# pauxy-qmc/pauxy

Measured on AMD Instinct MI355X. Metric: walker_steps_per_sec, higher is better.
Workload: dtype f64; 1 GPU; generic Cholesky AFQMC: Nbasis=100, Nchol=500, RHF trial 25+25 electrons, 256 walkers/GPU, dt=0.005, reortho/10, comb/5, energy/10 (BASELINE configs[2]); walkers_total=256, rng=device-philox, population_control=device comb (one rank)

## Files before the change

include/afqmc_hip.h:

```cpp
#ifndef AFQMC_HIP_H
#define AFQMC_HIP_H

#include <stdint.h>

#ifdef __cplusplus
extern "C" {
#endif

typedef struct afq_handle afq_handle;

#define AFQ_OK            0
#define AFQ_EINVAL       (-1)
#define AFQ_ESTATE       (-2)
#define AFQ_EHIP         (-3)
#define AFQ_ENOMEM       (-4)
#define AFQ_EUNSUPPORTED (-5)
#define AFQ_EWEIGHT      (-6)
#define AFQ_EOVERFLOW    (-7)
#define AFQ_ECOMM        (-8)

#define AFQ_SYS_GENERIC 1
#define AFQ_SYS_HUBBARD 2
#define AFQ_SYS_UEG     3

// ... 103 lines not shown
int afq_propagate_begin(afq_handle *h, const double *xi);
int afq_propagate_finish(afq_handle *h, double eshift_re, double eshift_im);
int afq_reortho(afq_handle *h, double *detR_out);
int afq_set_log_shift(afq_handle *h, int on, double log_shift, double detR_shift);
int afq_log_ovlp_sums(afq_handle *h, double *sums3);
int afq_local_energy(afq_handle *h, double *E_out);

int afq_set_exchange_algorithm(afq_handle *h, int mode);
int afq_exchange_algorithm(afq_handle *h, int *mode_out);

int afq_set_propagator_closed_form(afq_handle *h, int mode);
int afq_propagator_closed_form(afq_handle *h, int *mode_out);

int afq_set_step_fusion(afq_handle *h, int mode);
int afq_set_step_fusion_scope(afq_handle *h, int scope);

int afq_set_msd_force_bias(afq_handle *h, int mode);
int afq_msd_force_bias(afq_handle *h, int *mode_out);

int afq_force_bias(afq_handle *h, double *xbar_out);
int afq_shift_fields(afq_handle *h, const double *xi, const double *xbar,
                     double *xs_out, double *cmf_out, double *cfb_out);
int afq_vhs(afq_handle *h, const double *xs, double *vhs_out);
int afq_vhs_count(afq_handle *h, int *nv);
int afq_apply_exponential(afq_handle *h, const double *vhs);
int afq_kinetic(afq_handle *h);

int afq_cap_weights(afq_handle *h, double frac, double total_weight);
int afq_set_weight_cap(afq_handle *h, double frac, double total_weight);
int afq_popcontrol_comb(afq_handle *h, double r, double target_weight,
// ... 89 lines not shown
```

pauxy_amd/_lib.py:

```python
import ctypes
import os
from ctypes import POINTER, c_char_p, c_double, c_int, c_int32, c_int64, c_uint64, c_void_p

HERE = os.path.dirname(os.path.abspath(__file__))
LIB_PATH = os.environ.get("AFQ_LIBRARY") or os.path.join(HERE, "libafqmc_hip.so")

AFQ_OK = 0
AFQ_EWEIGHT, AFQ_EOVERFLOW, AFQ_ECOMM = -6, -7, -8
AFQ_COMM_NSTATS = 12
ALLGATHER_FN = ctypes.CFUNCTYPE(ctypes.c_int, ctypes.c_void_p, ctypes.c_void_p, ctypes.c_int, ctypes.c_void_p)
AFQ_SYS_GENERIC, AFQ_SYS_HUBBARD, AFQ_SYS_UEG = 1, 2, 3
AFQ_PROP_HYBRID, AFQ_PROP_FORCE_BIAS, AFQ_PROP_FREE_PROJECTION, AFQ_PROP_HUBBARD_SPIN = 1, 2, 4, 8
(F_PHI, F_WEIGHT, F_UNSCALED_WEIGHT, F_OT, F_HYBRID_ENERGY, F_PHASE, F_DETR, F_ELOC, F_GHALF, F_G,
 F_XBAR, F_XSHIFTED, F_ENERGY, F_LOG_DETR, F_THERMAL_G, F_THERMAL_STACK, F_THERMAL_RIGHT, F_THERMAL_M0,
 F_THERMAL_DET, F_CMF, F_CFB) = range(21)
THERMAL_CHARGE, THERMAL_FREE_PROJECTION, THERMAL_LOW_RANK, THERMAL_AVERAGE_GF = 1, 2, 4, 8
AFQ_EINVAL, AFQ_ESTATE, AFQ_EUNSUPPORTED = -1, -2, -5

_h = c_void_p
_dp = c_void_p
_ip = c_void_p

SIGNATURES = {
    "afq_version": [],
# ... 97 lines not shown
    "afq_comm_set_timeout": [_h, c_double],
    "afq_launch_trace": [_h, c_int],
    "afq_launch_trace_get": [_h, c_void_p, c_int, c_void_p, c_void_p, c_int, POINTER(c_int)],
    "afq_comm_stats": [_h, c_void_p],
    "afq_comm_parent_ix": [_h, c_void_p],
    "afq_estimates_allreduce": [_h, _dp, c_int],
    "afq_comm_init_local": [POINTER(_h), c_int],
    "afq_popcontrol_comb_local": [POINTER(_h), c_int, c_double, c_double, c_void_p, POINTER(c_double)],
    "afq_estimates_allreduce_local": [POINTER(_h), c_int],
    "afq_set_exchange_algorithm": [_h, c_int],
    "afq_exchange_algorithm": [_h, POINTER(c_int)],
    "afq_set_propagator_closed_form": [_h, c_int],
    "afq_propagator_closed_form": [_h, POINTER(c_int)],
    "afq_set_step_fusion": [_h, c_int],
    "afq_set_step_fusion_scope": [_h, c_int],
    "afq_set_msd_force_bias": [_h, c_int],
    "afq_msd_force_bias": [_h, POINTER(c_int)],
    "afq_kernel_trace": [_h, c_int],
    "afq_kernel_trace_stride": [_h, c_int, c_int],
    "afq_kernel_trace_get": [_h, c_int, _dp, c_int, POINTER(c_int)],
    "afq_kernel_issued_flops": [_h, c_int, POINTER(c_double)],
    "afq_thermal_configure": [_h, c_int, c_int, c_int, _dp, _dp, _dp, _dp, c_int],
    "afq_thermal_reset": [_h],
    "afq_thermal_propagate": [_h, _dp, c_void_p, c_double],
    "afq_thermal_greens": [_h, c_int],
    "afq_thermal_energy": [_h, _dp, _dp],
    "afq_thermal_state": [_h, c_void_p],
    "afq_thermal_configure_continuous": [_h, c_int, c_int, c_double, _dp, _dp, _dp, _dp, c_double, c_int],
    "afq_thermal_propagate_continuous": [_h, _dp, _dp],
}
# ... 41 lines not shown
```

pauxy_amd/csrc/afq_api.hip:

```cpp
#include <algorithm>
#include <cmath>
#include <complex>
#include <cstdio>
#include <cstdlib>
#include <cstring>
#include "afq_host.h"
#include "walker_fields.h"

namespace {

void free_dets(afq_handle *h) {
    h->mem.release(LT_TRIAL);
    h->dets.assign(1, afq_handle::DetOps());
    h->ndet = 1;
    select_det(h, 0, true);
    h->msd_fb_gbar = false;
}

void free_system(afq_handle *h) {
    free_dets(h);
    h->mem.release(LT_SYSTEM);
    h->hs_cplx = 0; h->sf_nlong = 0; h->kind = 0; h->pair_nb = 0;
    h->hirsch = false;
}
// ... 24 lines not shown
                const double hr = hrow[2 * q], hi = hrow[2 * q + 1];
                out[2 * q] += cr * hr - ci * hi;
                out[2 * q + 1] += cr * hi + ci * hr;
            }
        }
    }
    int rc = dev_upload(h, LT_TRIAL, &h->dets[h->cur_det].rH1, r.data(), (size_t)nt * M);
    select_det(h, h->cur_det, true);
    return rc;
}

}

struct afq_host_cache {
    std::vector<double> H1, psi;
};
static afq_host_cache *cache_of(afq_handle *h);

struct afq_handle_full : afq_handle {
    afq_host_cache cache;
};
static afq_host_cache *cache_of(afq_handle *h) { return &static_cast<afq_handle_full *>(h)->cache; }

static int upload_psi(afq_handle *h, const double *psi) {
    const size_t n = (size_t)h->M * h->nt;
    afq_handle::DetOps &o = h->dets[h->cur_det];
    int rc = dev_upload(h, LT_TRIAL, &o.psi, psi, n);
    if (rc) return rc;
    cache_of(h)->psi.assign(psi, psi + 2 * n);
    h->psi_real = true;
    for (size_t i = 0; i < n && h->psi_real; ++i) h->psi_real = psi[2 * i + 1] == 0.0;
    h->psi_closed = h->na == h->nb && h->na > 0;
    for (int p_ = 0; p_ < h->M && h->psi_closed; ++p_)
        h->psi_closed = memcmp(psi + 2 * (size_t)p_ * h->nt, psi + 2 * ((size_t)p_ * h->nt + h->na), sizeof(double) * 2 * h->na) == 0;
    std::vector<double> pc(psi, psi + 2 * n);
    for (size_t i = 0; i < n; ++i) pc[2 * i + 1] = -pc[2 * i + 1];
    if (h->ndet <= 1) {
        std::vector<double> pt(2 * n);
        for (int p_ = 0; p_ < h->M; ++p_)
            for (int i = 0; i < h->nt; ++i) {
                pt[2 * ((size_t)i * h->M + p_)] = pc[2 * ((size_t)p_ * h->nt + i)];
                pt[2 * ((size_t)i * h->M + p_) + 1] = pc[2 * ((size_t)p_ * h->nt + i) + 1];
            }
        if ((rc = dev_upload(h, LT_TRIAL, &h->psicT, pt.data(), n))) return rc;
    }
    rc = dev_upload(h, LT_TRIAL, &o.psic, pc.data(), n);
    select_det(h, h->cur_det, true);
    return rc;
}

static int maybe_build_rH1(afq_handle *h) {
    afq_host_cache *c = cache_of(h);
    if (h->kind == 0 || !h->have_trial || c->H1.empty()) return AFQ_OK;
    return build_rH1(h, c->H1, c->psi);
}

__global__ void afq_marker_kernel(volatile unsigned long long *retired, unsigned long long n) { *retired = n; }

void afq_launch_trace_mark(afq_handle *h, const char *name) {
    const size_t pairs = h->ltrace_name.size();
    if (name && pairs >= 65536) return;
    auto event_at = [&](size_t i) {
// ... 405 lines not shown
    }
    return AFQ_OK;
}

int afq_set_propagator(afq_handle *h, const double *BH1, const double *mf_shift, double dt, int exp_order,
                       int flags) {
    if (h) h->gf.drop();
    if (!h || !BH1 || !mf_shift || dt <= 0 || exp_order < 0) return AFQ_EINVAL;
    if (!h->kind) AFQ_FAIL(h, AFQ_ESTATE, "set the system before the propagator");
    hipSetDevice(h->device);
    int rc;
    if ((rc = dev_upload(h, LT_HANDLE, &h->BH1, BH1, (size_t)2 * h->M * h->M))) return rc;
    h->bh1_real = true;
    h->bh1_same = memcmp(BH1, BH1 + (size_t)2 * h->M * h->M, sizeof(double) * 2 * h->M * h->M) == 0;
    for (size_t i = 0, n = (size_t)2 * h->M * h->M; i < n && h->bh1_real; ++i) h->bh1_real = BH1[2 * i + 1] == 0.0;
    if ((rc = dev_upload(h, LT_HANDLE, &h->mf_shift, mf_shift, (size_t)h->K))) return rc;
    if (h->kind == AFQ_SYS_UEG && (rc = k_ueg_fast_propagator(h, BH1))) return rc;
    h->dt = dt; h->sqrt_dt = std::pow(dt, 0.5); h->exp_order = exp_order;
    if (flags & AFQ_PROP_FREE_PROJECTION) flags &= ~AFQ_PROP_FORCE_BIAS;
    const int old_nv = h->nv; const bool old_diag = h->vhs_diag;
    h->flags = flags;
    h->vhs_diag = h->kind == AFQ_SYS_HUBBARD;
    h->nv = (h->kind == AFQ_SYS_HUBBARD && (flags & AFQ_PROP_HUBBARD_SPIN)) ? 2 : 1;
    h->have_prop = true;
    if (h->nw && (old_nv != h->nv || old_diag != h->vhs_diag || !h->vhs)) {
        const size_t per = h->vhs_diag ? (size_t)2 * h->nv * h->M : (size_t)h->nv * h->M * h->M;
        if ((rc = dev_alloc(h, LT_WALKERS, &h->vhs, per * h->nw))) return rc;
    }
    return AFQ_OK;
}

int afq_walkers_alloc(afq_handle *h, int nw) {
    if (h) h->gf.drop();
    if (!h || nw <= 0) return AFQ_EINVAL;
    if (!h->kind) AFQ_FAIL(h, AFQ_ESTATE, "set the system before allocating walkers");
    hipSetDevice(h->device);
    free_walkers(h);
    const size_t per = (size_t)h->M * h->nt, K = h->K, n = nw;
    int rc = 0;
// ... 492 lines not shown
    return AFQ_OK;
}

int afq_set_step_fusion(afq_handle *h, int mode) {
    if (!h || mode < 0 || mode > 2) return AFQ_EINVAL;
    h->step_fusion_mode = mode;
    return AFQ_OK;
}

int afq_set_step_fusion_scope(afq_handle *h, int scope) {
    if (!h || scope < 0 || scope > 1) return AFQ_EINVAL;
    h->step_fusion_scope = scope;
    return AFQ_OK;
}

int afq_propagator_closed_form(afq_handle *h, int *mode) {
    if (!h || !mode) return AFQ_EINVAL;
    *mode = k_prop_closed_resident(h) ? 2 : 1;
    return AFQ_OK;
}

int afq_set_msd_force_bias(afq_handle *h, int mode) {
    if (!h || mode < 0 || mode > 2) return AFQ_EINVAL;
    h->msd_fb_mode = mode;
    return AFQ_OK;
}

int afq_msd_force_bias(afq_handle *h, int *mode) {
    if (!h || !mode) return AFQ_EINVAL;
    if (h->kind != AFQ_SYS_GENERIC || !h->have_trial || !h->nw) AFQ_FAIL(h, AFQ_ESTATE, "generic system, trial and walkers must be set");
// ... 517 lines not shown
    if (!h->hirsch) AFQ_FAIL(h, AFQ_ESTATE, "the discrete Hirsch propagator is not set");
    return hirsch_buffers(h);
}

int afq_set_propagator_hirsch(afq_handle *h, const double *bt2, double dt, int charge_decomposition) {
    if (h) h->gf.drop();
    if (!h || !bt2 || dt <= 0) return AFQ_EINVAL;
    if (h->kind != AFQ_SYS_HUBBARD) AFQ_FAIL(h, AFQ_ESTATE, "the Hirsch transformation needs a Hubbard system");
    if (h->ndet > 1) AFQ_FAIL(h, AFQ_EUNSUPPORTED, "Hirsch propagator: single-determinant trials");
    hipSetDevice(h->device);
    int rc;
    if ((rc = dev_upload(h, LT_HANDLE, &h->BH1, bt2, (size_t)2 * h->M * h->M))) return rc;
    h->bh1_real = true;
    for (size_t i = 0, n = (size_t)2 * h->M * h->M; i < n && h->bh1_real; ++i) h->bh1_real = bt2[2 * i + 1] == 0.0;
    h->bh1_same = false;
    typedef std::complex<double> C;
    C gamma, auxf[2][2], wfac[2];
    const double e = std::exp(-0.5 * dt * h->U);
    if (charge_decomposition) {
        gamma = std::acosh(C(e, 0.0));
        auxf[0][0] = auxf[0][1] = std::exp(gamma);
        auxf[1][0] = auxf[1][1] = std::exp(-gamma);
        wfac[0] = std::exp(0.5 * dt * h->U) * std::exp(-gamma);
        wfac[1] = std::exp(0.5 * dt * h->U) * std::exp(gamma);
    } else {
        gamma = C(std::acosh(std::exp(0.5 * dt * h->U)), 0.0);
        auxf[0][0] = std::exp(gamma); auxf[0][1] = std::exp(-gamma);
        auxf[1][0] = std::exp(-gamma); auxf[1][1] = std::exp(gamma);
        wfac[0] = wfac[1] = C(1.0, 0.0);
    }
// ... 189 lines not shown
```

pauxy_amd/csrc/afq_internal.h:

```cpp
#pragma once
#include <hip/hip_runtime.h>
#include <stdint.h>
#include <cstdlib>
#include <string>
#include <vector>
#include "../../include/afqmc_hip.h"
#include "greens_cache.h"
#include "dev_mem.h"

typedef double2 cplx;

__host__ __device__ inline cplx cmake(double r, double i) { return make_double2(r, i); }
__host__ __device__ inline cplx cadd(cplx a, cplx b) { return cmake(a.x + b.x, a.y + b.y); }
__host__ __device__ inline cplx csub(cplx a, cplx b) { return cmake(a.x - b.x, a.y - b.y); }
__host__ __device__ inline cplx cmul(cplx a, cplx b) {
    return cmake(a.x * b.x - a.y * b.y, a.x * b.y + a.y * b.x);
}
__host__ __device__ inline cplx cconj(cplx a) { return cmake(a.x, -a.y); }
__host__ __device__ inline cplx cscale(cplx a, double s) { return cmake(a.x * s, a.y * s); }
__host__ __device__ inline void cfma(cplx &a, cplx b, cplx c) {
    a.x = fma(b.x, c.x, a.x); a.x = fma(-b.y, c.y, a.x);
    a.y = fma(b.x, c.y, a.y); a.y = fma(b.y, c.x, a.y);
}
__host__ __device__ inline double cabs2(cplx a) { return a.x * a.x + a.y * a.y; }
__device__ inline cplx cdiv(cplx a, cplx b) {
    if (fabs(b.x) >= fabs(b.y)) {
        double r = b.y / b.x, d = b.x + b.y * r;
        return cmake((a.x + a.y * r) / d, (a.y - a.x * r) / d);
    } else {
        double r = b.x / b.y, d = b.x * r + b.y;
        return cmake((a.x * r + a.y) / d, (a.y * r - a.x) / d);
    }
}

#define AFQ_NSCAL 12
enum { AFQ_HS_HERMITIAN = 1, AFQ_HS_GENERAL = 2 };
enum { T_GREENS = 0, T_ONEBODY, T_FB, T_VHS, T_EXP, T_OVLP, T_QR, T_ENERGY, T_COUNT };

#define AFQ_NCOUNTERS 8

struct afq_handle {
    int device = 0;
    hipStream_t stream = nullptr;
    std::string err;
    DevMem mem;

    int kind = 0;
    int M = 0, K = 0, na = 0, nb = 0, nt = 0;
    double ecore = 0.0;
    double *hs_pot = nullptr;
    bool hs_sym = false;
    double *L_full = nullptr;
    int2 *hs_pair = nullptr;
    int hs_cplx = 0;
// ... 1 lines not shown
    int2 *hs_pair_im = nullptr;
    long ld_hs_im = 0;
    cplx *L_full_c = nullptr;
    long ld_hs = 0, ld_rc = 0;
    bool rchol_real = true;
    double *rchol_re = nullptr;
    double *rchol_im = nullptr;
    double *rchol_frag[2] = {nullptr, nullptr};
    double *rchol_frag_im[2] = {nullptr, nullptr};
    void *atil[2] = {nullptr, nullptr};
    bool atil_unavailable = false;
    bool rchol_same = false;
    int exx_mode = 0;
    int step_fusion_mode = 2;
    int step_fusion_scope = 0;
    int prop_closed_mode = 0;
    cplx *exq_y = nullptr;
    size_t exq_y_len = 0;
    cplx *H1 = nullptr;
    cplx *rH1 = nullptr;
    double U = 0.0;
    int nq = 0;
    int64_t nnzA = 0, nnzB = 0;
    int64_t *iA_colptr = nullptr, *iA_row = nullptr; cplx *iA_val = nullptr;
    int64_t *iB_colptr = nullptr, *iB_row = nullptr; cplx *iB_val = nullptr;
    int64_t *iA_rowptr = nullptr, *iA_col = nullptr; cplx *iA_rval = nullptr;
    int64_t *iB_rowptr = nullptr, *iB_col = nullptr; cplx *iB_rval = nullptr;
    int ell_len = 0; int *ell_row = nullptr; cplx *ell_val = nullptr;
    int ueg_nrows = 0; int *ueg_rmap = nullptr; int *ueg_rows = nullptr;
    int *ueg_kp = nullptr, *ueg_pm = nullptr, *ueg_koff = nullptr, *ueg_poff = nullptr;
// ... 7 lines not shown
    size_t sf_ws_len = 0, sf_two_len = 0;
    cplx *corr_ws = nullptr;
    size_t corr_ws_len = 0;
    int *pair_nbr = nullptr;
    int pair_nb = 0;
    cplx *pair_ws = nullptr;
    size_t pair_ws_len = 0;

    bool have_trial = false;
    cplx *psi = nullptr;
    cplx *psic = nullptr;
    cplx *psicT = nullptr;
    long psi_stride = 0;
    bool psi_real = false;
    bool psi_closed = false;
    unsigned long long *closed_bad = nullptr;
    unsigned long long closed_epoch = 0;
    unsigned long long closed_epoch_pub = 0;
    bool exx_open_hint = false;
    int *closed_w = nullptr;
    size_t closed_w_n = 0;
    bool closed_large = false;

    struct DetOps {
        cplx *psi = nullptr, *psic = nullptr, *rH1 = nullptr;
        double *rchol_re = nullptr, *rchol_im = nullptr;
        double *rchol_frag[2] = {nullptr, nullptr}, *rchol_frag_im[2] = {nullptr, nullptr};
        void *atil[2] = {nullptr, nullptr};
        bool rchol_same = false;
        GreensCache::Stamp vbias_stamp;
// ... 459 lines not shown
```

pauxy_amd/csrc/greens_small.h:

```cpp
#pragma once
#include <type_traits>
#include "mfma_gemm.h"
#include "gj_wave.h"
#include "lds_dma.h"
#include "weight_update.h"

struct GreensArgs {
    int M, na, nb, nt, nw;
    const cplx *phi, *psi;
    long psi_stride;
    cplx *ghalf;
    cplx *gsum;
    cplx *oinv;
    cplx *det;
    cplx *det_a;
    cplx *ws;
    int o_in_lds;
    int only_alive;
    const int *alive;
    int psi_real;
    int skip_spin;
    int psi_closed;
    unsigned long long *closed_bad;
    unsigned long long closed_epoch;
    unsigned long long *counters;
};

struct GreensLaunch {
    enum Path { BIG, SMALL, LU } path;
    GreensArgs a;
    WeightArgs wa;
    size_t lds;
    bool ride, inverse, wgj, tiny;
};

#define GS_KSMAX 32
template <bool INVERSE, bool WGJ>
__device__ __attribute__((always_inline)) inline void greens_small_body(const GreensArgs &a, const WeightArgs &wa, const int w,
                                                                       unsigned char *smem, const bool known_closed) {
    __shared__ cplx ph_s[2];
    __shared__ double la_s[2];
    __shared__ unsigned long long pmax_s[2][48];
    const int tid = threadIdx.x;
    const int g = __builtin_amdgcn_readfirstlane(tid >> 8), wave = __builtin_amdgcn_readfirstlane((tid >> 6) & 3);
    const int lane = tid & 63;
    unsigned long long *pmax = pmax_s[g];
    if ((tid & 255) < 48) pmax[tid & 255] = 0ull;
    const int M = a.M, nt = a.nt;
    const int nmax = a.na > a.nb ? a.na : a.nb;
    const int n = g == 0 ? a.na : a.nb, off = g == 0 ? 0 : a.na;
    cplx *O = (cplx *)smem + (long)g * (nmax * nmax + 2 * nmax);
    cplx *colk = O + nmax * nmax, *rowk = colk + nmax;
    int *piv = (int *)((cplx *)smem + 2L * (nmax * nmax + 2 * nmax)) + g * nmax;
    cplx *phi_l = (cplx *)smem + 2L * (nmax * nmax + 2 * nmax) + ((2 * nmax + 3) / 4 + 1);
// ... 94 lines not shown
                    mf(xa, gq);
                }
                if (gq + 1 < ng) {
                    if (gq + 2 < ng) readx(xa, gq + 2 < NG ? gq + 2 : 0);
                    mf(xb, gq + 1);
                }
            }
#pragma unroll
            for (int r = 0; r < 4; ++r) {
                const int i = ti * 16 + lk + 4 * r, j = tj * 16 + lr;
                if (i < n && j < n) O[i * n + j] = YR ? cmake(accR[r], acc3[r]) : cmake(accR[r] + accI[r], acc3[r] - accR[r] + accI[r]);
            }
            if (WGJ) break;
        }
    };
    if (yreal) phase01(std::true_type{});
    else phase01(std::false_type{});
    __syncthreads();
    __shared__ cplx gj_row[2][32], gj_piv[2][32];
    __shared__ int gj_prow[2][32];
    if (WGJ) {
        if (wave == g && !(closed && g == 1)) {
            cplx ph;
            int la;
            gj_wave32(O, n, lane, INVERSE, gj_row[g], gj_piv[g], gj_prow[g], ph, la);
            if (lane == 0) {
                ph_s[g] = ph; la_s[g] = (double)la;
                if (closed) { ph_s[1] = ph; la_s[1] = (double)la; }
            }
        }
    } else if (wave == 0) {
        cplx ph = cmake(1.0, 0.0);
        int la = 0;
        const int cw_shift = n <= 32 ? 5 : 6;
        const int cj = lane & ((1 << cw_shift) - 1), ri = lane >> cw_shift, rstep = 64 >> cw_shift;
        for (int k = 0; k < n; ++k) {
            unsigned long long mbits = 0;
// ... 191 lines not shown
```

pauxy_amd/csrc/k_fused.hip:

```cpp
#include <cstdlib>
#include <type_traits>

#include "mfma_gemm_wg.h"
#include "greens_small.h"

#define PF_D 3
#ifndef PF_NW
#define PF_NW 8
#endif
#define PF_NT (64 * PF_NW)
#ifndef PF_LW
#define PF_LW PF_NW
#endif
#define PF_FPW (16 / PF_LW)

struct PropFusedArgs {
    int M, na, nb, nt, order;
    int vhs_upper;
    int same_b;
    int b_real;
    int rem4;
    int hyb;
    int symcols;
    int closed_try;
// ... 46 lines not shown
}

__device__ inline void lds_barrier() {
    asm volatile("s_waitcnt lgkmcnt(0)" ::: "memory");
    __builtin_amdgcn_s_barrier();
    asm volatile("" ::: "memory");
}

#include "k_fused_closed.h"

template <bool NARROW, int FULL>
__global__ __launch_bounds__(PF_NT) void prop_fused_kernel(PropFusedArgs a) {
    extern __shared__ __align__(16) unsigned char smem[];
    constexpr bool MUL3 = false;
#define PF_LEAVE(stored_closed_) return
#include "k_fused_body.h"
#undef PF_LEAVE
}

template <bool NARROW, int FULL, bool TAIL, bool MUL3>
__global__ __launch_bounds__(PF_NT) void prop_fused_kernel(PropFusedArgs a, GreensArgs ga, WeightArgs wa) {
    static_assert(TAIL && !NARROW && FULL == 7, "the tail rides on the full wide deal only");
    extern __shared__ __align__(16) unsigned char smem[];
    bool stored_closed = false;
    do {
#define PF_LEAVE(stored_closed_) { stored_closed = (stored_closed_); break; }
#include "k_fused_body.h"
#undef PF_LEAVE
    } while (0);
    asm volatile("s_waitcnt vmcnt(0) lgkmcnt(0)" ::: "memory");
    __syncthreads();
    int w = blockIdx.x;
    asm volatile("" : "+s"(w));
    greens_small_body<true, true>(ga, wa, w, smem, stored_closed);
}

int k_prop_fused_supported(afq_handle *h) {
    return !h->vhs_diag && h->nv == 1 && h->M <= 104 && h->na <= 32 && h->nb <= 32 && h->nb > 0;
}

int k_prop_closed_resident(afq_handle *h) {
    return PF_NW == 8 && k_prop_fused_supported(h) && h->prop_closed_mode != 1 && h->bh1_same && h->bh1_real &&
           h->na == h->nb && h->na > 16 && h->na <= 32 && h->M > 96 && h->M <= 104 && h->exp_order > 0;
}

int k_step_fusion_shape(afq_handle *h) {
    if (!k_prop_closed_resident(h)) return 0;
    const size_t nmax = h->na, NCH = (h->M + 7) / 8;
    const size_t tail = sizeof(cplx) * (2 * (nmax * nmax + 2 * nmax) + ((2 * nmax + 3) / 4 + 1) + (size_t)h->M * h->nt);
// ... 9 lines not shown
    a.rem4 = (h->M > 96 && h->M <= 100) ? 1 : 0;
    a.hyb = 0;
    a.contig = 0; a.symcols = 0;
    if (a.rem4 && a.same_b && h->na > 16 && h->nb > 16 && h->nt > 48 && h->nt <= 56 && PF_NW == 8) {
        a.contig = 1;
        a.hyb = (h->nt - 48 + 3) / 4;
    }
    a.symcols = (a.contig && h->na == h->nb) ? 1 : 0;
    a.closed_try = 0;
    a.BH1 = h->BH1; a.vhs = h->vhs; a.phi = h->phi; a.alive = h->alive; a.zero16 = h->zero_page;
    a.n_closed = h->counters + 3;
    const int NCH = (h->M + 7) / 8;
    const size_t lds = (size_t)NCH * 8192 + (size_t)PF_D * 16384;
    static size_t lds_set[8][AFQ_MAX_DEVICES] = {{0}, {0}, {0}, {0}, {0}, {0}, {0}, {0}};
    const bool narrow = h->na <= 16 && h->nb <= 16;
    KernelTrace kt(h, AFQ_K_PROPAGATOR);
    {
        const int nrt_ = (h->M + 15) / 16, ct = (h->na + 15) / 16 + (h->nb + 15) / 16;
        const double ksteps = 2.0 * NCH;
        const double per_pass = ksteps * (2048.0 * (a.rem4 ? nrt_ - 1 : nrt_) * ct + 512.0 * (a.rem4 ? ct : 0));
        const double taylor_pass = a.contig ? ksteps * (2048.0 * (nrt_ - 1) * 3 + 512.0 * (nrt_ - 1) * a.hyb + 512.0 * 4) : per_pass;
        h->issued_flops[AFQ_K_PROPAGATOR] = (3.0 * h->exp_order * taylor_pass + 2.0 * (a.b_real ? 2.0 : 3.0) * per_pass) * h->nw;
        h->prop_issued_open = h->issued_flops[AFQ_K_PROPAGATOR] / h->nw;
        const int cta = (h->na + 15) / 16;
        const double closed_pass = ksteps * (2048.0 * (a.rem4 ? nrt_ - 1 : nrt_) * cta + 512.0 * (a.rem4 ? cta : 0));
        h->prop_issued_closed = 3.0 * h->exp_order * closed_pass + 2.0 * (a.b_real ? 2.0 : 3.0) * per_pass;
        if (k_prop_closed_resident(h))
            h->prop_issued_closed = ((tail && mul3 ? 3.0 : 4.0) * h->exp_order + 2.0 * 2.0) * ((h->M + 3) / 4) * 2048.0 * 7 * 2;
        if (tail) {
            const double t16 = (h->na + 15) / 16, m16 = (h->M + 15) / 16;
            const double ks1 = 4.0 * (((h->M + 3) / 4 + 3) / 4), ks3 = (h->na + 3) / 4;
            const double spin = 2048.0 * (t16 * t16 * ks1 * (tail->a.psi_real ? 2.0 : 3.0) + t16 * m16 * ks3 * 3.0);
            h->prop_issued_open += 2.0 * spin;
            h->prop_issued_closed += (tail->a.psi_closed ? 1.0 : 2.0) * spin;
            h->issued_flops[AFQ_K_PROPAGATOR] = h->prop_issued_open * h->nw;
        }
    }
    const int nrt = (h->M + 15) / 16;
    const bool nofull = PF_NW != 8;
    const int full = nofull ? 0 : narrow ? (nrt == 6 ? 6 : 0) : (nrt >= 5 && h->na > 16 && h->nb > 16 ? nrt : 0);
    a.closed_try = (a.same_b && h->na == h->nb && h->exp_order > 0 && full != 0 && PF_NW == 8 &&
                    (!a.contig || a.symcols)) ? 1 : 0;
    a.resident = (a.closed_try && full == 7 && k_prop_closed_resident(h)) ? 1 : 0;
#define PF_LAUNCH_(NARROW_, FULL_, SLOT_)                                                                     \
    do {                                                                                                      \
        AFQ_HIP(h, afq_raise_lds((const void *)prop_fused_kernel<NARROW_, FULL_>, lds, lds_set[SLOT_]));      \
        AFQ_LAUNCH(h, (prop_fused_kernel<NARROW_, FULL_>), dim3(h->nw), dim3(PF_NT), lds, h->stream, a);      \
    } while (0)
    if (tail) {
        if (full != 7 || !a.resident || tail->lds > lds)
            AFQ_FAIL(h, AFQ_ESTATE, "internal: a Green's function tail on a propagator launch outside its shape class");
        if (mul3) {
            AFQ_HIP(h, afq_raise_lds((const void *)prop_fused_kernel<false, 7, true, true>, lds, lds_set[6]));
            AFQ_LAUNCH(h, (prop_fused_kernel<false, 7, true, true>), dim3(h->nw), dim3(PF_NT), lds, h->stream, a, tail->a, tail->wa);
        } else {
            AFQ_HIP(h, afq_raise_lds((const void *)prop_fused_kernel<false, 7, true, false>, lds, lds_set[7]));
            AFQ_LAUNCH(h, (prop_fused_kernel<false, 7, true, false>), dim3(h->nw), dim3(PF_NT), lds, h->stream, a, tail->a, tail->wa);
        }
    }
    else if (narrow && full) PF_LAUNCH_(true, 6, 0);
    else if (narrow) PF_LAUNCH_(true, 0, 1);
    else if (full == 7) PF_LAUNCH_(false, 7, 2);
    else if (full == 6) PF_LAUNCH_(false, 6, 3);
    else if (full == 5) PF_LAUNCH_(false, 5, 4);
    else PF_LAUNCH_(false, 0, 5);
#undef PF_LAUNCH_
    AFQ_POST(h);
    return AFQ_OK;
}
```

pauxy_amd/csrc/k_fused_body.h:

```cpp
    const int w = blockIdx.x;
    if (!a.alive[w]) PF_LEAVE(false);
    const int tid = threadIdx.x, lane = tid & 63, wave = __builtin_amdgcn_readfirstlane(tid >> 6);
    const int lr = lane & 15, lk = lane >> 4;
    const int M = a.M, nt = a.nt;
    const int NCH = (M + 7) >> 3;
    const int nrt = (M + 15) >> 4;
    unsigned char *Tf = smem;
    unsigned char *ring = smem + (size_t)NCH * 8192;
    const unsigned tf_l = lds_addr(Tf), ring_l = lds_addr(ring);
    cplx *phi = a.phi + (long)w * M * nt;
    const cplx *vhs = a.vhs + (long)w * M * M;

    const int nob = a.same_b ? 1 : 2;
    const int nphase = 2 * nob + a.order;
    const int G = nphase * NCH;
    const long MM = (long)M * M;
    int gi = 0, gi_phase = 0, gi_c = 0, gi_slot = 0;
    const void *nsrc[PF_FPW];
    bool prepared = false;
    const bool refills = wave >= PF_NW - PF_LW;
    const int lw = wave - (PF_NW - PF_LW);
    const int p_row0 = (lw >> 1) * 16 + lr;
    const int p_kl = 2 * lk + (lw & 1);
    auto prepare = [&]() __attribute__((always_inline)) {
// ... 32 lines not shown
    if (a.closed_try) {
        bool same = true;
        for (int p = tid >> 5; p < M; p += PF_NT / 32) {
            const int c = tid & 31;
            if (c < a.na) {
                const cplx x = phi[p * nt + c], y = phi[p * nt + a.na + c];
                same = same && __double_as_longlong(x.x) == __double_as_longlong(y.x) &&
                       __double_as_longlong(x.y) == __double_as_longlong(y.y);
            }
        }
        closed = __builtin_amdgcn_readfirstlane(__syncthreads_and(same ? 1 : 0)) != 0;
        if (closed && tid == 0) atomicAdd(a.n_closed, 1ULL);
    }
    if constexpr (!NARROW && FULL == 7 && PF_NW == 8) {
        if (closed && a.resident) {
            if (M <= 100) prop_closed_resident<25, MUL3>(a, smem, phi, vhs);
            else prop_closed_resident<26, MUL3>(a, smem, phi, vhs);
            PF_LEAVE(true);
        }
    }
    const bool relayout = closed && a.contig;
    const int contig = relayout ? 0 : a.contig, hyb = relayout ? 0 : a.hyb;
    const int sym_n = (a.symcols && !relayout) ? a.na : 0;
    auto wcol = [&](const int c) -> int {
        if (!sym_n) return c;
        if (c < 16) return c;
        if (c < 32) return sym_n + (c - 16);
        if (c < 40) return 16 + (c - 32);
        if (c < 48) return sym_n + 16 + (c - 40);
        const int e = c - 48, extra = sym_n - 24;
        return e < extra ? 24 + e : sym_n + 24 + (e - extra);
    };
// ... 798 lines not shown
```

pauxy_amd/csrc/k_fused_closed.h:

```cpp
#pragma once

#define PCR_LDS(p) ((__attribute__((address_space(3))) unsigned char *)(p))

template <int KS, bool MUL3>
__device__ __attribute__((always_inline)) inline void prop_closed_resident(const PropFusedArgs &a, unsigned char *smem_,
                                                                           cplx *phi, const cplx *vhs) {
    auto *smem = PCR_LDS(smem_);
    typedef __attribute__((address_space(3))) d2_t lds_d2;
    const int tid = threadIdx.x, wave = __builtin_amdgcn_readfirstlane(tid >> 6);
    const int M = a.M, nt = a.nt, na = a.na;
    constexpr unsigned TB = KS * 2048;
    const bool mul = wave < 7;
    auto lane_id = [&]() __attribute__((always_inline)) -> int {
        int t = tid;
        asm volatile("" : "+v"(t));
        return t & 63;
    };

    for (int e = tid; e < KS * 128; e += PF_NT) {
        const int k = 4 * (e >> 7) + ((e >> 4) & 3), col = 16 * ((e >> 6) & 1) + (e & 15);
        const bool ok = k < M && col < na;
        const cplx v = phi[ok ? k * nt + col : 0];
        ((lds_d2 *)smem)[e] = ok ? (d2_t){v.x, v.y} : (d2_t){0.0, 0.0};
    }
    __syncthreads();

    auto load_b = [&](double (&bh)[KS]) __attribute__((always_inline)) {
        const int lane = lane_id(), lk = lane >> 4, row = wave * 16 + (lane & 15);
#pragma unroll
        for (int s = 0; s < KS; ++s) {
            const int k = 4 * s + lk;
            const double *p = (row < M && k < M) ? &a.BH1[row * M + k].x : (const double *)a.zero16;
            bh[s] = *p;
        }
    };
    auto one_body = [&](const unsigned src, const double (&bh)[KS], d4_t (&P1)[2], d4_t (&P2)[2]) __attribute__((always_inline)) {
#pragma unroll
        for (int j = 0; j < 2; ++j) { P1[j] = (d4_t){0, 0, 0, 0}; P2[j] = (d4_t){0, 0, 0, 0}; }
// ... 19 lines not shown
    };

    d2_t av[KS];
    d4_t SR[2], SI[2];
    if (mul) {
        double bh[KS];
        load_b(bh);
        const int lane = lane_id(), lk = lane >> 4, row = wave * 16 + (lane & 15);
#pragma unroll
        for (int s = 0; s < KS; ++s) {
            const int k = 4 * s + lk;
            const int off = (a.vhs_upper && k < row) ? k * M + row : row * M + k;
            const d2_t *p = (row < M && k < M) ? (const d2_t *)(vhs + off) : (const d2_t *)a.zero16;
            av[s] = *p;
        }
        one_body(0, bh, SR, SI);
        put(TB, SR, SI);
    }
    lds_barrier();

    unsigned cur = TB;
    for (int n = 1; n <= a.order; ++n) {
        if (mul) {
            double inv_n = 1.0 / n;
            asm volatile("" : "+v"(inv_n));
            d4_t P1[2], P2[2], P3[2];
#pragma unroll
            for (int j = 0; j < 2; ++j) { P1[j] = (d4_t){0, 0, 0, 0}; P2[j] = (d4_t){0, 0, 0, 0}; P3[j] = (d4_t){0, 0, 0, 0}; }
            const auto *tb = smem + cur + lane_id() * 16;
#pragma unroll
            for (int s = 0; s < KS; ++s) {
                asm volatile("" : "+v"(av[s]));
#pragma unroll
                for (int j = 0; j < 2; ++j) {
                    const d2_t b = *(const lds_d2 *)(tb + (s * 2 + j) * 1024);
                    if constexpr (MUL3) {
// ... 12 lines not shown
#pragma unroll
            for (int j = 0; j < 2; ++j)
#pragma unroll
                for (int q = 0; q < 4; ++q) {
                    re[j][q] = (P1[j][q] - P2[j][q]) * inv_n;
                    im[j][q] = (MUL3 ? P3[j][q] - P1[j][q] - P2[j][q] : P3[j][q]) * inv_n;
                    SR[j][q] += re[j][q]; SI[j][q] += im[j][q];
                }
            if (n == a.order) put(cur ^ TB, SR, SI);
            else put(cur ^ TB, re, im);
        }
        lds_barrier();
        cur ^= TB;
    }

    if (mul) {
        d4_t P1[2], P2[2];
        double bh[KS];
        load_b(bh);
        one_body(cur, bh, P1, P2);
        const int lane = lane_id(), lr = lane & 15, lk = lane >> 4;
#pragma unroll
        for (int j = 0; j < 2; ++j)
#pragma unroll
            for (int q = 0; q < 4; ++q) {
                const int orow = wave * 16 + lk + 4 * q, col = 16 * j + lr;
                if (orow < M && col < na) {
                    const cplx v = cmake(P1[j][q], P2[j][q]);
                    phi[(long)orow * nt + col] = v;
                    phi[(long)orow * nt + na + col] = v;
// ... 5 lines not shown
```

pauxy_amd/device.py:

```python
import ctypes

import numpy

from pauxy_amd import _lib as L


def _c128(a, shape=None):
    a = numpy.ascontiguousarray(a, dtype=numpy.complex128)
    if shape is not None:
        assert a.shape == tuple(shape), (a.shape, shape)
    return a


def _f64(a, shape=None):
    a = numpy.ascontiguousarray(a, dtype=numpy.float64)
    if shape is not None:
        assert a.shape == tuple(shape), (a.shape, shape)
    return a


def _i64(a):
    return numpy.ascontiguousarray(a, dtype=numpy.int64)


# ... 676 lines not shown

    def exchange_algorithm(self):
        m = ctypes.c_int()
        self._ck(self.lib.afq_exchange_algorithm(self.h, ctypes.byref(m)))
        return m.value

    def set_propagator_closed_form(self, mode):
        self._ck(self.lib.afq_set_propagator_closed_form(self.h, int(mode)))

    def set_step_fusion(self, mode):
        self._ck(self.lib.afq_set_step_fusion(self.h, int(mode)))

    def set_step_fusion_scope(self, scope):
        self._ck(self.lib.afq_set_step_fusion_scope(self.h, int(scope)))

    def propagator_closed_form(self):
        m = ctypes.c_int()
        self._ck(self.lib.afq_propagator_closed_form(self.h, ctypes.byref(m)))
        return m.value

    def set_msd_force_bias(self, mode):
        self._ck(self.lib.afq_set_msd_force_bias(self.h, int(mode)))

    def msd_force_bias(self):
        m = ctypes.c_int()
        self._ck(self.lib.afq_msd_force_bias(self.h, ctypes.byref(m)))
        return m.value


def _handle_array(devs):
# ... 34 lines not shown
```

Baseline: 1.147 million walker-steps/s.

## Overlap Green's tail with final propagator one-body step via precomputed psi^T·B

Precomputes psiB = psi^T·exp(-dt H1/2) on the host for real closed-shell single-determinant trials. Inside the fused propagator kernel, the overlap matrix is then formed from the pre-kinetic walker state, and one wave runs the Gauss-Jordan inverse while the other waves run the final one-body multiply. The following Green's tail skips its own overlap build and inversion phases, taking phase and log-amplitude from the early result. This reorders the work to cut serial phases and barriers in the tail, at the cost of extra LDS staging, a host-side precompute and more template paths.

```diff
diff --git a/include/afqmc_hip.h b/include/afqmc_hip.h
--- a/include/afqmc_hip.h
+++ b/include/afqmc_hip.h
@@ -141,6 +141,7 @@
 
 int afq_set_step_fusion(afq_handle *h, int mode);
 int afq_set_step_fusion_scope(afq_handle *h, int scope);
+int afq_set_step_tail_overlap(afq_handle *h, int on);
 
 int afq_set_msd_force_bias(afq_handle *h, int mode);
 int afq_msd_force_bias(afq_handle *h, int *mode_out);
diff --git a/pauxy_amd/_lib.py b/pauxy_amd/_lib.py
--- a/pauxy_amd/_lib.py
+++ b/pauxy_amd/_lib.py
@@ -135,6 +135,7 @@
     "afq_propagator_closed_form": [_h, POINTER(c_int)],
     "afq_set_step_fusion": [_h, c_int],
     "afq_set_step_fusion_scope": [_h, c_int],
+    "afq_set_step_tail_overlap": [_h, c_int],
     "afq_set_msd_force_bias": [_h, c_int],
     "afq_msd_force_bias": [_h, POINTER(c_int)],
     "afq_kernel_trace": [_h, c_int],
diff --git a/pauxy_amd/csrc/afq_api.hip b/pauxy_amd/csrc/afq_api.hip
--- a/pauxy_amd/csrc/afq_api.hip
+++ b/pauxy_amd/csrc/afq_api.hip
@@ -62,6 +62,7 @@
 
 struct afq_host_cache {
     std::vector<double> H1, psi;
+    std::vector<double> BH1;
 };
 static afq_host_cache *cache_of(afq_handle *h);
 
@@ -69,6 +70,8 @@
     afq_host_cache cache;
 };
 static afq_host_cache *cache_of(afq_handle *h) { return &static_cast<afq_handle_full *>(h)->cache; }
+
+static int build_psiB(afq_handle *h);
 
 static int upload_psi(afq_handle *h, const double *psi) {
     const size_t n = (size_t)h->M * h->nt;
@@ -94,6 +97,26 @@
     }
     rc = dev_upload(h, LT_TRIAL, &o.psic, pc.data(), n);
     select_det(h, h->cur_det, true);
+    return rc ? rc : build_psiB(h);
+}
+
+static int build_psiB(afq_handle *h) {
+    afq_host_cache *c = cache_of(h);
+    const int M = h->M, nt = h->nt, na = h->na;
+    const bool ok = h->have_prop && h->ndet <= 1 && h->psi_stride == 0 && h->psi_real && h->psi_closed &&
+                    h->bh1_real && h->bh1_same && c->psi.size() == (size_t)2 * M * nt && c->BH1.size() == (size_t)M * M;
+    h->psiB_psi = nullptr; h->psiB_bh1 = nullptr;
+    if (!ok) return dev_alloc(h, LT_TRIAL, &h->psiB_cT, 0);
+    std::vector<double> pb((size_t)na * M, 0.0);
+    for (int m = 0; m < M; ++m)
+        for (int i = 0; i < na; ++i) {
+            const double p = c->psi[2 * ((size_t)m * nt + i)];
+            const double *brow = &c->BH1[(size_t)m * M];
+            double *out = &pb[(size_t)i * M];
+            for (int k = 0; k < M; ++k) out[k] += p * brow[k];
+        }
+    const int rc = dev_upload(h, LT_TRIAL, &h->psiB_cT, pb.data(), pb.size());
+    if (!rc) { h->psiB_psi = h->dets[h->cur_det].psi; h->psiB_bh1 = h->BH1; }
     return rc;
 }
 
@@ -529,6 +552,11 @@
     h->bh1_real = true;
     h->bh1_same = memcmp(BH1, BH1 + (size_t)2 * h->M * h->M, sizeof(double) * 2 * h->M * h->M) == 0;
     for (size_t i = 0, n = (size_t)2 * h->M * h->M; i < n && h->bh1_real; ++i) h->bh1_real = BH1[2 * i + 1] == 0.0;
+    {
+        std::vector<double> &b = cache_of(h)->BH1;
+        b.resize((size_t)h->M * h->M);
+        for (size_t i = 0; i < b.size(); ++i) b[i] = BH1[2 * i];
+    }
     if ((rc = dev_upload(h, LT_HANDLE, &h->mf_shift, mf_shift, (size_t)h->K))) return rc;
     if (h->kind == AFQ_SYS_UEG && (rc = k_ueg_fast_propagator(h, BH1))) return rc;
     h->dt = dt; h->sqrt_dt = std::pow(dt, 0.5); h->exp_order = exp_order;
@@ -538,6 +566,7 @@
     h->vhs_diag = h->kind == AFQ_SYS_HUBBARD;
     h->nv = (h->kind == AFQ_SYS_HUBBARD && (flags & AFQ_PROP_HUBBARD_SPIN)) ? 2 : 1;
     h->have_prop = true;
+    if ((rc = build_psiB(h))) return rc;
     if (h->nw && (old_nv != h->nv || old_diag != h->vhs_diag || !h->vhs)) {
         const size_t per = h->vhs_diag ? (size_t)2 * h->nv * h->M : (size_t)h->nv * h->M * h->M;
         if ((rc = dev_alloc(h, LT_WALKERS, &h->vhs, per * h->nw))) return rc;
@@ -1060,6 +1089,12 @@
     return AFQ_OK;
 }
 
+int afq_set_step_tail_overlap(afq_handle *h, int on) {
+    if (!h || on < 0 || on > 1) return AFQ_EINVAL;
+    h->step_tail_overlap = on;
+    return AFQ_OK;
+}
+
 int afq_propagator_closed_form(afq_handle *h, int *mode) {
     if (!h || !mode) return AFQ_EINVAL;
     *mode = k_prop_closed_resident(h) ? 2 : 1;
@@ -1607,6 +1642,8 @@
     h->bh1_real = true;
     for (size_t i = 0, n = (size_t)2 * h->M * h->M; i < n && h->bh1_real; ++i) h->bh1_real = bt2[2 * i + 1] == 0.0;
     h->bh1_same = false;
+    cache_of(h)->BH1.clear();
+    if ((rc = build_psiB(h))) return rc;
     typedef std::complex<double> C;
     C gamma, auxf[2][2], wfac[2];
     const double e = std::exp(-0.5 * dt * h->U);
diff --git a/pauxy_amd/csrc/afq_internal.h b/pauxy_amd/csrc/afq_internal.h
--- a/pauxy_amd/csrc/afq_internal.h
+++ b/pauxy_amd/csrc/afq_internal.h
@@ -37,7 +37,7 @@
 enum { AFQ_HS_HERMITIAN = 1, AFQ_HS_GENERAL = 2 };
 enum { T_GREENS = 0, T_ONEBODY, T_FB, T_VHS, T_EXP, T_OVLP, T_QR, T_ENERGY, T_COUNT };
 
-#define AFQ_NCOUNTERS 8
+#define AFQ_NCOUNTERS 9
 
 struct afq_handle {
     int device = 0;
@@ -69,6 +69,7 @@
     int exx_mode = 0;
     int step_fusion_mode = 2;
     int step_fusion_scope = 0;
+    int step_tail_overlap = 1;
     int prop_closed_mode = 0;
     cplx *exq_y = nullptr;
     size_t exq_y_len = 0;
@@ -106,6 +107,8 @@
     long psi_stride = 0;
     bool psi_real = false;
     bool psi_closed = false;
+    double *psiB_cT = nullptr;
+    const void *psiB_psi = nullptr, *psiB_bh1 = nullptr;
     unsigned long long *closed_bad = nullptr;
     unsigned long long closed_epoch = 0;
     unsigned long long closed_epoch_pub = 0;
diff --git a/pauxy_amd/csrc/greens_small.h b/pauxy_amd/csrc/greens_small.h
--- a/pauxy_amd/csrc/greens_small.h
+++ b/pauxy_amd/csrc/greens_small.h
@@ -35,9 +35,16 @@
 };
 
 #define GS_KSMAX 32
-template <bool INVERSE, bool WGJ>
+struct EarlyTail {
+    bool on;
+    cplx ph;
+    int la;
+};
+
+template <bool INVERSE, bool WGJ, bool EARLY = false>
 __device__ __attribute__((always_inline)) inline void greens_small_body(const GreensArgs &a, const WeightArgs &wa, const int w,
-                                                                       unsigned char *smem, const bool known_closed) {
+                                                                       unsigned char *smem, const bool known_closed,
+                                                                       const EarlyTail *early = nullptr) {
     __shared__ cplx ph_s[2];
     __shared__ double la_s[2];
     __shared__ unsigned long long pmax_s[2][48];
@@ -162,13 +169,20 @@
             if (WGJ) break;
         }
     };
-    if (yreal) phase01(std::true_type{});
+    bool skip012 = false;
+    if constexpr (EARLY) skip012 = early->on;
+    if (skip012) {
+        closed = true;
+        if (tid == 0 && a.counters) { atomicAdd(&a.counters[5], 1ull); atomicAdd(&a.counters[8], 1ull); }
+        if (tid == 448) { ph_s[0] = early->ph; ph_s[1] = early->ph; la_s[0] = (double)early->la; la_s[1] = (double)early->la; }
+    }
+    else if (yreal) phase01(std::true_type{});
     else phase01(std::false_type{});
-    __syncthreads();
+    if (!skip012) __syncthreads();
     __shared__ cplx gj_row[2][32], gj_piv[2][32];
     __shared__ int gj_prow[2][32];
     if (WGJ) {
-        if (wave == g && !(closed && g == 1)) {
+        if (wave == g && !(closed && g == 1) && !skip012) {
             cplx ph;
             int la;
             gj_wave32(O, n, lane, INVERSE, gj_row[g], gj_piv[g], gj_prow[g], ph, la);
diff --git a/pauxy_amd/csrc/k_fused.hip b/pauxy_amd/csrc/k_fused.hip
--- a/pauxy_amd/csrc/k_fused.hip
+++ b/pauxy_amd/csrc/k_fused.hip
@@ -84,25 +84,38 @@
     extern __shared__ __align__(16) unsigned char smem[];
     constexpr bool MUL3 = false;
 #define PF_LEAVE(stored_closed_) return
+#define PF_RESIDENT(KS_) prop_closed_resident<KS_, MUL3>(a, smem, phi, vhs)
 #include "k_fused_body.h"
+#undef PF_RESIDENT
 #undef PF_LEAVE
 }
 
 template <bool NARROW, int FULL, bool TAIL, bool MUL3>
-__global__ __launch_bounds__(PF_NT) void prop_fused_kernel(PropFusedArgs a, GreensArgs ga, WeightArgs wa) {
+__global__ __launch_bounds__(PF_NT) void prop_fused_kernel(PropFusedArgs a, GreensArgs ga, WeightArgs wa, const double *psiB) {
     static_assert(TAIL && !NARROW && FULL == 7, "the tail rides on the full wide deal only");
     extern __shared__ __align__(16) unsigned char smem[];
     bool stored_closed = false;
+    EarlyTail early;
+    early.on = false;
     do {
 #define PF_LEAVE(stored_closed_) { stored_closed = (stored_closed_); break; }
+#define PF_RESIDENT(KS_)                                                                                      \
+    do {                                                                                                      \
+        if constexpr (MUL3) {                                                                                 \
+            if (psiB) prop_closed_resident<KS_, true, true>(a, smem, phi, vhs, psiB, &early);                 \
+            else prop_closed_resident<KS_, true>(a, smem, phi, vhs);                                          \
+        } else prop_closed_resident<KS_, false>(a, smem, phi, vhs);                                           \
+    } while (0)
 #include "k_fused_body.h"
+#undef PF_RESIDENT
 #undef PF_LEAVE
     } while (0);
     asm volatile("s_waitcnt vmcnt(0) lgkmcnt(0)" ::: "memory");
     __syncthreads();
     int w = blockIdx.x;
     asm volatile("" : "+s"(w));
-    greens_small_body<true, true>(ga, wa, w, smem, stored_closed);
+    if constexpr (MUL3) greens_small_body<true, true, true>(ga, wa, w, smem, stored_closed, &early);
+    else greens_small_body<true, true>(ga, wa, w, smem, stored_closed);
 }
 
 int k_prop_fused_supported(afq_handle *h) {
@@ -142,6 +155,10 @@
     const size_t lds = (size_t)NCH * 8192 + (size_t)PF_D * 16384;
     static size_t lds_set[8][AFQ_MAX_DEVICES] = {{0}, {0}, {0}, {0}, {0}, {0}, {0}, {0}};
     const bool narrow = h->na <= 16 && h->nb <= 16;
+    const bool early = tail && mul3 && h->step_tail_overlap && h->psiB_cT && k_prop_closed_resident(h) &&
+                       tail->a.psi_real && tail->a.psi_closed && tail->a.psi_stride == 0 &&
+                       (const void *)tail->a.psi == h->psiB_psi && (const void *)h->BH1 == h->psiB_bh1 &&
+                       tail->a.gsum && tail->a.ghalf && !tail->a.oinv;
     KernelTrace kt(h, AFQ_K_PROPAGATOR);
     {
         const int nrt_ = (h->M + 15) / 16, ct = (h->na + 15) / 16 + (h->nb + 15) / 16;
@@ -161,6 +178,7 @@
             const double spin = 2048.0 * (t16 * t16 * ks1 * (tail->a.psi_real ? 2.0 : 3.0) + t16 * m16 * ks3 * 3.0);
             h->prop_issued_open += 2.0 * spin;
             h->prop_issued_closed += (tail->a.psi_closed ? 1.0 : 2.0) * spin;
+            if (early) h->prop_issued_closed += 2048.0 * (4.0 * ((h->M + 3) / 4) * 2.0 - t16 * t16 * ks1 * 2.0);
             h->issued_flops[AFQ_K_PROPAGATOR] = h->prop_issued_open * h->nw;
         }
     }
@@ -180,10 +198,12 @@
             AFQ_FAIL(h, AFQ_ESTATE, "internal: a Green's function tail on a propagator launch outside its shape class");
         if (mul3) {
             AFQ_HIP(h, afq_raise_lds((const void *)prop_fused_kernel<false, 7, true, true>, lds, lds_set[6]));
-            AFQ_LAUNCH(h, (prop_fused_kernel<false, 7, true, true>), dim3(h->nw), dim3(PF_NT), lds, h->stream, a, tail->a, tail->wa);
+            const double *psiB = early ? h->psiB_cT : nullptr;
+            AFQ_LAUNCH(h, (prop_fused_kernel<false, 7, true, true>), dim3(h->nw), dim3(PF_NT), lds, h->stream, a, tail->a, tail->wa, psiB);
         } else {
+            const double *psiB = nullptr;
             AFQ_HIP(h, afq_raise_lds((const void *)prop_fused_kernel<false, 7, true, false>, lds, lds_set[7]));
-            AFQ_LAUNCH(h, (prop_fused_kernel<false, 7, true, false>), dim3(h->nw), dim3(PF_NT), lds, h->stream, a, tail->a, tail->wa);
+            AFQ_LAUNCH(h, (prop_fused_kernel<false, 7, true, false>), dim3(h->nw), dim3(PF_NT), lds, h->stream, a, tail->a, tail->wa, psiB);
         }
     }
     else if (narrow && full) PF_LAUNCH_(true, 6, 0);
diff --git a/pauxy_amd/csrc/k_fused_body.h b/pauxy_amd/csrc/k_fused_body.h
--- a/pauxy_amd/csrc/k_fused_body.h
+++ b/pauxy_amd/csrc/k_fused_body.h
@@ -70,8 +70,8 @@
     }
     if constexpr (!NARROW && FULL == 7 && PF_NW == 8) {
         if (closed && a.resident) {
-            if (M <= 100) prop_closed_resident<25, MUL3>(a, smem, phi, vhs);
-            else prop_closed_resident<26, MUL3>(a, smem, phi, vhs);
+            if (M <= 100) PF_RESIDENT(25);
+            else PF_RESIDENT(26);
             PF_LEAVE(true);
         }
     }
diff --git a/pauxy_amd/csrc/k_fused_closed.h b/pauxy_amd/csrc/k_fused_closed.h
--- a/pauxy_amd/csrc/k_fused_closed.h
+++ b/pauxy_amd/csrc/k_fused_closed.h
@@ -2,11 +2,13 @@
 
 #define PCR_LDS(p) ((__attribute__((address_space(3))) unsigned char *)(p))
 
-template <int KS, bool MUL3>
+template <int KS, bool MUL3, bool EARLY = false>
 __device__ __attribute__((always_inline)) inline void prop_closed_resident(const PropFusedArgs &a, unsigned char *smem_,
-                                                                           cplx *phi, const cplx *vhs) {
+                                                                           cplx *phi, const cplx *vhs,
+                                                                           const double *psiB = nullptr, EarlyTail *et = nullptr) {
     auto *smem = PCR_LDS(smem_);
     typedef __attribute__((address_space(3))) d2_t lds_d2;
+    typedef __attribute__((address_space(3))) double lds_f64;
     const int tid = threadIdx.x, wave = __builtin_amdgcn_readfirstlane(tid >> 6);
     const int M = a.M, nt = a.nt, na = a.na;
     constexpr unsigned TB = KS * 2048;
@@ -17,11 +19,12 @@
         return t & 63;
     };
 
+    const unsigned base0 = (EARLY && (a.order & 1)) ? TB : 0u;
     for (int e = tid; e < KS * 128; e += PF_NT) {
         const int k = 4 * (e >> 7) + ((e >> 4) & 3), col = 16 * ((e >> 6) & 1) + (e & 15);
         const bool ok = k < M && col < na;
         const cplx v = phi[ok ? k * nt + col : 0];
-        ((lds_d2 *)smem)[e] = ok ? (d2_t){v.x, v.y} : (d2_t){0.0, 0.0};
+        ((lds_d2 *)(smem + base0))[e] = ok ? (d2_t){v.x, v.y} : (d2_t){0.0, 0.0};
     }
     __syncthreads();
 
@@ -71,12 +74,32 @@
             const d2_t *p = (row < M && k < M) ? (const d2_t *)(vhs + off) : (const d2_t *)a.zero16;
             av[s] = *p;
         }
-        one_body(0, bh, SR, SI);
-        put(TB, SR, SI);
+        one_body(base0, bh, SR, SI);
+        put(base0 ^ TB, SR, SI);
+    }
+    constexpr unsigned PB = 2 * TB;
+    if constexpr (EARLY) {
+        if (!mul) {
+            const int lane = lane_id(), lk = lane >> 4, lr = lane & 15;
+            double pv[2][KS];
+#pragma unroll
+            for (int t = 0; t < 2; ++t)
+#pragma unroll
+                for (int s = 0; s < KS; ++s) {
+                    const int j = 16 * t + lr, k = 4 * s + lk;
+                    const double *p = (j < na && k < M) ? psiB + j * M + k : (const double *)a.zero16;
+                    pv[t][s] = *p;
+                }
+            auto *pb = smem + PB + lane * 8;
+#pragma unroll
+            for (int t = 0; t < 2; ++t)
+#pragma unroll
+                for (int s = 0; s < KS; ++s) *(lds_f64 *)(pb + (t * KS + s) * 512) = pv[t][s];
+        }
     }
     lds_barrier();
 
-    unsigned cur = TB;
+    unsigned cur = base0 ^ TB;
     for (int n = 1; n <= a.order; ++n) {
         if (mul) {
             double inv_n = 1.0 / n;
@@ -119,6 +142,68 @@
         cur ^= TB;
     }
 
+    if constexpr (EARLY) {
+        const int nn = na, nsq = nn * nn + 2 * nn;
+        cplx *O = (cplx *)smem_;
+        cplx *phi_l = (cplx *)smem_ + 2L * nsq + ((2 * nn + 3) / 4 + 1);
+        {
+            const int t = wave >> 2, j = (wave >> 1) & 1, part = wave & 1;
+            const auto *pa = smem + PB + t * (KS * 512) + lane_id() * 8;
+            const auto *tb = smem + cur + j * 1024 + part * 8 + lane_id() * 16;
+            d4_t acc0 = {0, 0, 0, 0}, acc1 = {0, 0, 0, 0};
+#pragma unroll
+            for (int s = 0; s < KS; ++s) {
+                const double x = *(const lds_f64 *)(pa + s * 512), y = *(const lds_f64 *)(tb + s * 2048);
+                if (s & 1) acc1 = mfma16(x, y, acc1);
+                else acc0 = mfma16(x, y, acc0);
+            }
+            const int lane = lane_id(), lr = lane & 15, lk = lane >> 4;
+#pragma unroll
+            for (int q = 0; q < 4; ++q) {
+                const int i = 16 * j + lr, jj = 16 * t + 4 * q + lk;
+                if (i < nn && jj < nn) ((double *)&O[i * nn + jj])[part] = acc0[q] + acc1[q];
+            }
+        }
+        lds_barrier();
+        d4_t P1[2], P2[2];
+        if (mul) {
+            double bh[KS];
+            load_b(bh);
+            one_body(cur, bh, P1, P2);
+            const int lane = lane_id(), lr = lane & 15, lk = lane >> 4;
+#pragma unroll
+            for (int j = 0; j < 2; ++j)
+#pragma unroll
+                for (int q = 0; q < 4; ++q) {
+                    const int orow = wave * 16 + lk + 4 * q, col = 16 * j + lr;
+                    if (orow < M && col < na) {
+                        const cplx v = cmake(P1[j][q], P2[j][q]);
+                        phi[(long)orow * nt + col] = v;
+                        phi[(long)orow * nt + na + col] = v;
+                    }
+                }
+        } else {
+            cplx *scr = O + nsq;
+            gj_wave32(O, nn, lane_id(), true, scr, scr + 32, (int *)(scr + 64), et->ph, et->la);
+        }
+        lds_barrier();
+        if (mul) {
+            const int lane = lane_id(), lr = lane & 15, lk = lane >> 4;
+#pragma unroll
+            for (int j = 0; j < 2; ++j)
+#pragma unroll
+                for (int q = 0; q < 4; ++q) {
+                    const int orow = wave * 16 + lk + 4 * q, col = 16 * j + lr;
+                    if (orow < M && col < na) {
+                        const cplx v = cmake(P1[j][q], P2[j][q]);
+                        phi_l[orow * nt + col] = v;
+                        phi_l[orow * nt + na + col] = v;
+                    }
+                }
+        }
+        et->on = true;
+        return;
+    }
     if (mul) {
         d4_t P1[2], P2[2];
         double bh[KS];
diff --git a/pauxy_amd/device.py b/pauxy_amd/device.py
--- a/pauxy_amd/device.py
+++ b/pauxy_amd/device.py
@@ -714,6 +714,9 @@
     def set_step_fusion_scope(self, scope):
         self._ck(self.lib.afq_set_step_fusion_scope(self.h, int(scope)))
 
+    def set_step_tail_overlap(self, on):
+        self._ck(self.lib.afq_set_step_tail_overlap(self.h, int(on)))
+
     def propagator_closed_form(self):
         m = ctypes.c_int()
         self._ck(self.lib.afq_propagator_closed_form(self.h, ctypes.byref(m)))
```

Measured after the change: 1.186 million walker-steps/s (median of 6 runs). +3.4%, better.
